# jordi-adell/mcarray

Hardware: AMD Instinct MI355X
Metric: STFT frames/sec, 8-mic GCC-PHAT + SRP-PHAT(361) + delay-and-sum beamform @48kHz/1024-pt (higher is better)
Workload: dtype f32 (SRP operands adaptive); 1 GPU; BASELINE configs[2] geometry (8-mic ULA 0.04 m, 48 kHz, N=1024, hop 512, 361 angles, 1 source, no power floor), 8 arrays x 4096 frames per GPU per step; channel rows padded by 64 floats; arrays_per_gpu=8, frames_per_array=4096, srp_precision=adaptive, parallelism=arrays sharded over 1 GPU(s), all_gather of DOA bins+prob

## Files before the change

__graft_entry__.py:

```python
import os
import subprocess
import sys

ROOT = os.path.dirname(os.path.abspath(__file__))
if ROOT not in sys.path:
    sys.path.insert(0, ROOT)


def build():
    env = dict(os.environ)
    subprocess.check_call(["make", "-C", os.path.join(ROOT, "mcarray_amd", "csrc"), "-j4", "-s"], env=env)
    subprocess.check_call(["make", "-C", os.path.join(ROOT, "oracle"), "-s"], env=env)
    cxx = os.path.join(ROOT, "tests", "cxx", "Makefile")
    if os.path.exists(cxx):
        subprocess.check_call(["make", "-C", os.path.dirname(cxx), "-s"], env=env)
    import mcarray_amd
    from mcarray_amd import _lib
    _lib.load()


def smoke():
    import numpy as np
    from mcarray_amd import api, synth
    from oracle import pyoracle as po
    fs, N, F = 48000, 1024, 12
    xs = synth.ULA8
    pcm = synth.noise_source_stream(xs, np.deg2rad(23.0), fs, (F + 1) * N // 2, 42)
    ctx = api.Context(fs, xs, N, 0.5, 1, srp_precision=api.SRP_FP32, device=0)
    r = ctx.process_frames_host(pcm[None], want_energy=True)
    o = po.ssl_stream(fs, N, xs, pcm.astype(np.float64), 1, 0.5, want_map=True)
    assert np.array_equal(r["bin"][0], o["bin"]), (r["bin"][0].T, o["bin"].T)
    assert np.abs(r["energy"][0] - o["energy"]).max() <= 2e-5 * np.abs(o["energy"]).max()
    assert np.abs(r["out"][0] - o["out"]).max() <= 2e-5 * np.abs(o["out"]).max() + 1e-7
    print("smoke ok: DOA bins", r["bin"][0, :, 0].tolist(), "->", float(np.rad2deg(r["doa"][0, -1, 0])), "deg")


if __name__ == "__main__":
    build()
    if len(sys.argv) > 1 and sys.argv[1] == "smoke":
        smoke()
```

mcarray_amd/csrc/api.hip:

```cpp
#include "../../include/mcarray_hip.h"
#include "fft1024c.h"
#include "kernels.h"
#include "knobs.h"
#include "stage.h"

#include <chrono>
#include <cmath>
#include <cstdio>
#include <cstdlib>
#include <cstring>
#include <string>
#include <thread>
#include <vector>

using namespace mca;

namespace {

std::string g_create_error;

struct TimedEvent { int id; hipEvent_t a, b; };

}

struct mca_hip_graph;

#define MCA_MAX_LANES 1

constexpr int FB_LAG = 2, FB_RING = 64, FB_WAIT_MS = 4000;
struct Knobs {
    bool fb_enabled = true;
    long long adapt_min_rows = 4096;
    int adapt_max_sources = 1;
    double tau_scale = 1.0;
// ... 28 lines not shown
    {
        auto F = [](void *q) { if (q) (void)hipFree(q); };
        F(d_A); F(d_Ax); F(d_C); F(d_Cx); F(d_part); F(d_estart); F(d_nv); F(d_power); F(d_voiced); F(d_power_out);
        F(d_flags); F(d_chunk_from); F(d_list); F(d_need); F(d_umask); F(d_nlist); F(d_last_vchunk); F(d_unsure);
        *this = Workspace();
    }
};

struct G2FrameState {
    double power_floor = 0, samples = 0, noise_estimated = 0;
    double silence = 0;
    double corr_mem = 0, doa_mem = 0;
    double doa = 0, prob = -1;
};

struct mca_hip_ctx {
    mca_hip_config cfg{};
    std::vector<double> xyz;
    int M = 0, P = 0, G = 0, D = 0, Dp = 0, K = 0, N = 0, H = 0, logH = 0, Kp = 0, S = 1, prec = 0;
    bool ula = false, stream_ok = false, generic = false;
    bool n512 = false;
    bool n2048 = false;
    std::string stream_why;
    float step = 0.f;
    std::vector<float> delays, grid;
    std::vector<int2> pairs;
    float *d_window = nullptr, *d_grid = nullptr, *d_delays = nullptr;
    float2 *d_tw = nullptr;
    double *d_micx = nullptr;
    int2 *d_pairs = nullptr;
    void *d_B = nullptr, *d_Bt = nullptr;
    bool merged = false; int n_merged = 0, Kp_m = 0;
    void *d_Bm = nullptr, *d_Btm = nullptr; unsigned short *d_mrank = nullptr;
    float2 *d_bftab = nullptr; int bf_pairs = 0;
    float4 *d_steer_rows = nullptr; float2 *d_steer_q = nullptr; float *d_steer_nyq = nullptr; int *d_steer_pred = nullptr; unsigned long long *d_steer_miss = nullptr;
    float2 *d_steer_Y = nullptr; size_t steer_Y_rows = 0; float *d_steer_tail = nullptr;
    int *d_steer_mlist = nullptr;
    bool steer_now = false, steer_fused_now = false;
    bool steer_mlist_dirty = false;
    bool steer_patched_now = false;
    unsigned long long steer_frames_total = 0, steer_fused_calls = 0;
    unsigned long long *h_steer = nullptr;
    unsigned long long steer_seq = 0, steer_seq_seen = 0, steer_call_frames[FB_RING] = {};
    bool steer_spec = true, steer_lost = false;
    float *d_E[2] = {nullptr, nullptr};
    float *d_tail[2] = {nullptr, nullptr};
    int e_cur = 0, tail_cur = 0;
    Workspace lanes[MCA_MAX_LANES];
    int cur_lane = 0, a0 = 0;
    long long plan_rows = 0;
    int plan_arrays = 0;
    int n_lanes_last = 1;
    hipStream_t io_stream[3] = {}; hipEvent_t io_ev[8] = {};
    Workspace &ws() { return lanes[cur_lane]; }
    double *d_gate_state = nullptr;
    int *d_last_bin = nullptr; float *d_last_rad = nullptr, *d_last_prob = nullptr;
    int last_arrays = 0, last_frames = 0;
    float *d_doa[2] = {nullptr, nullptr};
    int doa_cur = 0;
    long long gcc2_frames_done = 0;
    long long *d_vdone[2] = {nullptr, nullptr};
    int *d_g2_vidx = nullptr, *d_g2_nv = nullptr; float *d_g2_rad = nullptr, *d_g2_prob = nullptr; size_t g2_rows = 0;
    unsigned char *d_g2_reset = nullptr;
    int *d_g2_post0 = nullptr;
    int *d_silence = nullptr;
    bool tracked = false;
// ... 51 lines not shown
namespace {

int fail(mca_hip_ctx *c, int code, const std::string &msg)
{
    if (c) c->err = msg; else g_create_error = msg;
    return code;
}

#define HIP_TRY(ctx, expr)                                                                              \
    do {                                                                                                \
        hipError_t _e = (expr);                                                                         \
        if (_e != hipSuccess)                                                                           \
            return fail(ctx, _e == hipErrorOutOfMemory ? MCA_HIP_ERR_OUT_OF_MEMORY : MCA_HIP_ERR_HIP,   \
                        std::string(#expr) + ": " + hipGetErrorString(_e));                            \
    } while (0)

double speed_of_sound() { return 346.1; }
float doa_idx2angle(int idx, float step) { float pr = (float)idx * step; return (float)((double)pr - M_PI_2); }
float doa_to_delay_far_field(float doa, float microDist)
{
    return (float)(((double)microDist * std::sin((double)doa)) / speed_of_sound());
}
float doa_to_delay_samples(float doa, float microDist, int fs) { return doa_to_delay_far_field(doa, microDist) * (float)fs; }
double distance(const std::vector<double> &xyz, int i, int j)
{
    return std::sqrt(std::pow(xyz[3 * j] - xyz[3 * i], 2) + std::pow(xyz[3 * j + 1] - xyz[3 * i + 1], 2) +
                     std::pow(xyz[3 * j + 2] - xyz[3 * i + 2], 2));
}

void free_ctx(mca_hip_ctx *c)
{
    if (!c) return;
    auto F = [](void *p) { if (p) (void)hipFree(p); };
    F(c->d_window); F(c->d_tw); F(c->d_grid); F(c->d_delays); F(c->d_micx); F(c->d_pairs); F(c->d_B); F(c->d_Bt); F(c->d_bftab); F(c->d_steer_rows); F(c->d_steer_q); F(c->d_steer_nyq); F(c->d_steer_pred); F(c->d_steer_miss); F(c->d_steer_Y); F(c->d_steer_mlist); F(c->d_steer_tail); F(c->d_Bm); F(c->d_Btm); F(c->d_mrank);
    F(c->d_E[0]); F(c->d_E[1]); F(c->d_tail[0]); F(c->d_tail[1]); F(c->d_doa[0]); F(c->d_doa[1]); F(c->d_vdone[0]); F(c->d_vdone[1]); F(c->d_g2_vidx); F(c->d_g2_nv); F(c->d_g2_rad); F(c->d_g2_prob);
    F(c->d_g2_reset); F(c->d_g2_post0); F(c->d_silence);
    F(c->d_trk_x); F(c->d_trk_sd); F(c->d_trk_si); F(c->d_trk_sil); F(c->d_trk_corr); F(c->d_trk_idx); F(c->d_trk_res);
    F(c->d_rstats); F(c->d_gate_state);
    for (int i = 0; i < 2; ++i) { F(c->d_hist_pcm[i]); F(c->d_hist_C[i]); F(c->d_ehist[i]); }
    if (c->h_probe) (void)hipHostFree(c->h_probe);
    if (c->h_steer) (void)hipHostFree(c->h_steer);
    for (Workspace &w : c->lanes) w.release();
    for (auto &e : c->io_ev) if (e) (void)hipEventDestroy(e);
    for (auto &q : c->io_stream) if (q) (void)hipStreamDestroy(q);
    F(c->d_last_bin); F(c->d_last_rad); F(c->d_last_prob);
    F(c->d_fr); F(c->d_E64[0]); F(c->d_E64[1]); F(c->d_res); F(c->d_bins); F(c->d_out64);
    F(c->d_g2f_corr[0]); F(c->d_g2f_corr[1]); F(c->d_g2f_res);
    c->stage.release();
    for (auto &e : c->events) { (void)hipEventDestroy(e.a); (void)hipEventDestroy(e.b); }
    for (auto &e : c->pool) (void)hipEventDestroy(e);
    delete c;
}

int round_up(int v, int m) { return (v + m - 1) / m * m; }

Knobs read_knobs(const mca_hip_config &cfg)
{
    Knobs k;
    auto geti = [](const char *v, long long dflt) { return v ? std::atoll(v) : dflt; };
    k.fb_enabled = cfg.adaptive_fallback != MCA_HIP_ADAPT_FALLBACK_OFF;
    if (const char *v = env_str("MCA_HIP_ADAPT_FALLBACK")) k.fb_enabled = std::atoi(v) != 0;
    k.adapt_min_rows = geti(env_str("MCA_HIP_ADAPT_MIN_ROWS"), cfg.adaptive_min_rows > 0 ? cfg.adaptive_min_rows : 4096);
    k.adapt_max_sources = (int)geti(env_str("MCA_HIP_ADAPT_MAX_SOURCES"), cfg.adaptive_max_sources > 0 ? cfg.adaptive_max_sources : 1);
    if (const char *v = env_str("MCA_HIP_ADAPT_TAU_SCALE")) k.tau_scale = std::atof(v);
    if (const char *v = env_str("MCA_HIP_WS_MAX_MB")) k.ws_max_bytes = (long long)std::atoll(v) << 20;
    k.force_generic = env_str("MCA_HIP_FORCE_GENERIC") != nullptr;
    k.scan_carry = cfg.scan_carry != 0 || env_str("MCA_HIP_SCAN_CARRY") != nullptr;
// ... 47 lines not shown
                        _Float16 hi = (_Float16)v[q];
                        B[(size_t)d * Kp + kk] = hi;
                        if (planes == 2) B[((size_t)Dp + d) * Kp + kk] = (_Float16)(v[q] - (float)hi);
                    }
                }
        HIP_TRY(c, hipMalloc(&c->d_B, B.size() * sizeof(_Float16)));
        HIP_TRY(c, hipMemcpy(c->d_B, B.data(), B.size() * sizeof(_Float16), hipMemcpyHostToDevice));
        if (Dp == 384) {
            const int ns32 = Kp / 32;
            std::vector<_Float16> Bt(B.size());
            for (int pl = 0; pl < planes; ++pl)
                for (int sl = 0; sl < ns32; ++sl)
                    for (int d = 0; d < Dp; ++d)
                        std::memcpy(&Bt[(((size_t)pl * ns32 + sl) * Dp + d) * 32], &B[((size_t)pl * Dp + d) * Kp + (size_t)sl * 32], 32 * sizeof(_Float16));
            HIP_TRY(c, hipMalloc(&c->d_Bt, Bt.size() * sizeof(_Float16)));
            HIP_TRY(c, hipMemcpy(c->d_Bt, Bt.data(), Bt.size() * sizeof(_Float16), hipMemcpyHostToDevice));
        }
    }
    return MCA_HIP_OK;
}

int cur_kp(const mca_hip_ctx *c) { return (c->merged && c->a_planes == 1) ? c->Kp_m : c->Kp; }

int build_merged_tables(mca_hip_ctx *c)
{
    c->merged = false;
    if (!c->ula || (c->generic && !c->n2048) || c->n512 || (c->M != 4 && c->M != 8) || c->Dp % 64 != 0) return MCA_HIP_OK;
    if (c->prec != MCA_HIP_SRP_ADAPTIVE && c->prec != MCA_HIP_SRP_FP16) return MCA_HIP_OK;
    const int K = c->K, D = c->D, Dp = c->Dp, G = c->G;
    const double N = 2.0 * (K - 1);
    for (int g = 1; g < G; ++g)
        for (int d = 0; d < D; ++d)
            if (std::fabs((double)c->delays[(size_t)g * D + d] - (g + 1) * (double)c->delays[d]) > 1e-4) return MCA_HIP_OK;
    std::vector<unsigned short> rank((size_t)G * (K - 1) + 1, 0xffff);
    std::vector<int> ms;
    for (int g = 1; g <= G; ++g)
        for (int k = 0; k < K; ++k) rank[(size_t)k * g] = 0;
    for (size_t m = 0; m < rank.size(); ++m)
        if (rank[m] == 0) { rank[m] = (unsigned short)ms.size(); ms.push_back((int)m); }
    c->n_merged = (int)ms.size();
    c->Kp_m = round_up(2 * ((c->n_merged + 63) & ~63), 32);
    const int Kp = c->Kp_m;
    std::vector<_Float16> B((size_t)Dp * Kp, (_Float16)0.f);
    for (int d = 0; d < D; ++d)
        for (int r = 0; r < c->n_merged; ++r) {
            const double ph = 2.0 * M_PI * (double)ms[(size_t)r] * (double)c->delays[d] / N;
            B[(size_t)d * Kp + 2 * r] = (_Float16)(float)std::cos(ph);
            B[(size_t)d * Kp + 2 * r + 1] = (_Float16)(float)(-std::sin(ph));
        }
    HIP_TRY(c, hipMalloc(&c->d_Bm, B.size() * sizeof(_Float16)));
    HIP_TRY(c, hipMemcpy(c->d_Bm, B.data(), B.size() * sizeof(_Float16), hipMemcpyHostToDevice));
    if (Dp == 384) {
        const int ns32 = Kp / 32;
        std::vector<_Float16> Bt(B.size());
        for (int sl = 0; sl < ns32; ++sl)
            for (int d = 0; d < Dp; ++d)
                std::memcpy(&Bt[((size_t)sl * Dp + d) * 32], &B[(size_t)d * Kp + (size_t)sl * 32], 32 * sizeof(_Float16));
        HIP_TRY(c, hipMalloc(&c->d_Btm, Bt.size() * sizeof(_Float16)));
        HIP_TRY(c, hipMemcpy(c->d_Btm, Bt.data(), Bt.size() * sizeof(_Float16), hipMemcpyHostToDevice));
    }
    rank.resize((rank.size() + 3) / 4 * 4, 0xffff);
    HIP_TRY(c, hipMalloc((void **)&c->d_mrank, rank.size() * sizeof(unsigned short)));
    HIP_TRY(c, hipMemcpy(c->d_mrank, rank.data(), rank.size() * sizeof(unsigned short), hipMemcpyHostToDevice));
    c->merged = true;
    c->a_row_elems = cur_kp(c) * c->a_planes;
    return MCA_HIP_OK;
}

void time_begin(mca_hip_ctx *c, int id, hipStream_t st)
{
    c->timing_open = (c->timing >> id) & 1u;
    if (!c->timing_open) return;
    TimedEvent ev; ev.id = id;
    auto get = [&]() { hipEvent_t e; if (!c->pool.empty()) { e = c->pool.back(); c->pool.pop_back(); } else (void)hipEventCreate(&e); return e; };
    ev.a = get(); ev.b = get();
    (void)hipEventRecord(ev.a, st);
    c->events.push_back(ev);
}
void time_end(mca_hip_ctx *c, hipStream_t st)
{
    if (!c->timing_open) return;
    c->timing_open = false;
    (void)hipEventRecord(c->events.back().b, st);
}

int gen_threads(const mca_hip_ctx *c, bool synthesis)
{
    if (c->N >= 4096) return 1024;
    if (c->N >= 2048) return synthesis ? 512 : 1024;
    return 256;
}

struct GemmPlan { bool v2; int ksplit; };
GemmPlan plan_gemm(const mca_hip_ctx *c, long long rows)
{
    GemmPlan g;
    if (c->plan_rows > 0) rows = c->plan_rows;
    const long long deep = cur_kp(c) >= 12288 ? 2 : 1;
    g.v2 = c->prec != MCA_HIP_SRP_FP32 && c->Dp == 384 && rows * (c->a_planes == 2 ? deep : 1) >= 16384LL * (c->a_planes == 2 ? 2 : 1);
    if (g.v2) {
        g.ksplit = rows >= 65536 ? 1 : (rows >= 32768 || cur_kp(c) < 6144 ? 2 : 4);
    } else {
        const long long wgs = (rows + 127) / 128 * (c->Dp == 64 ? 1 : c->Dp / 192);
        const int nk = cur_kp(c) / (c->prec == MCA_HIP_SRP_FP32 ? 16 : 32);
        long long ks = 512 / (wgs > 0 ? wgs : 1);
        if (ks > nk / 8) ks = nk / 8;
        if (ks > 16) ks = 16;
        if (ks < 1) ks = 1;
        g.ksplit = (int)ks;
    }
    return g;
}

void *&a_buf(mca_hip_ctx *c) { return (c->prec == MCA_HIP_SRP_ADAPTIVE && c->a_planes == 2) ? c->ws().d_Ax : c->ws().d_A; }
size_t &a_buf_bytes(mca_hip_ctx *c) { return (c->prec == MCA_HIP_SRP_ADAPTIVE && c->a_planes == 2) ? c->ws().ax_bytes : c->ws().a_bytes; }

int ensure_a(mca_hip_ctx *c, long long rows)
{
    size_t need_a = (size_t)((rows + 255) / 256 * 256) * c->a_row_elems * c->a_elem;
    void *&buf = a_buf(c); size_t &bytes = a_buf_bytes(c);
    if (need_a > bytes) {
        if (buf) (void)hipFree(buf);
        buf = nullptr; bytes = 0;
        HIP_TRY(c, hipMalloc(&buf, need_a));
        HIP_TRY(c, hipMemset(buf, 0, need_a));
        HIP_TRY(c, hipDeviceSynchronize());
        bytes = need_a; ++c->ws_gen;
    }
    return MCA_HIP_OK;
}

int ensure_workspace(mca_hip_ctx *c, long long rows_chunk, long long rows_total)
{
    int rc_a = ensure_a(c, rows_chunk);
    if (rc_a) return rc_a;
    const int planes = std::max(2, plan_gemm(c, rows_chunk).ksplit);
    size_t need_c = (size_t)rows_total * c->Dp * sizeof(float) * planes;
    if (need_c > c->ws().c_bytes) {
        if (c->ws().d_C) (void)hipFree(c->ws().d_C);
        c->ws().d_C = nullptr; c->ws().c_bytes = 0;
        HIP_TRY(c, hipMalloc((void **)&c->ws().d_C, need_c));
        c->ws().c_bytes = need_c; ++c->ws_gen;
    }
// ... 795 lines not shown
    c->cur_lane = 0;
    return reserve_lane(c, n_arrays, n_frames);
}

int mca_hip_reserve(mca_hip_ctx *c, int n_arrays, int n_frames)
{
    if (!c || n_arrays < 1 || n_frames < 1) return MCA_HIP_ERR_INVALID_ARGUMENT;
    const int rc = reserve_impl(c, n_arrays, n_frames);
    return rc ? rc : steer_reserve(c, n_arrays, n_frames);
}

static int run_correlation_map(mca_hip_ctx *c, const float *pcm, long long array_stride, long long mic_stride,
                               int n_arrays, int n_frames, hipStream_t st)
{
    int rc;
    const long long fc = chunk_frames_for(c, n_arrays, n_frames);
    if ((rc = ensure_workspace(c, (long long)n_arrays * fc, (long long)n_arrays * n_frames))) return rc;
    if ((rc = ensure_scan_workspace(c, n_arrays, n_frames, (n_frames + SCAN_CHUNK - 1) / SCAN_CHUNK))) return rc;
    bool fused_partial = SCAN_CHUNK == 32 && c->a_planes == 1 && !c->cfg.use_power_floor && n_frames % SCAN_CHUNK == 0 && fc % SCAN_CHUNK == 0 &&
                         plan_gemm(c, (long long)n_arrays * fc).ksplit <= 2;
    for (int f0 = 0; fused_partial && f0 < n_frames; f0 += (int)fc)
        fused_partial = plan_gemm(c, (long long)n_arrays * std::min<long long>(fc, n_frames - f0)).v2;
    c->ws().partial_done = fused_partial;
    c->ws().part_planes = fused_partial ? plan_gemm(c, (long long)n_arrays * fc).ksplit : 1;
    for (int f0 = 0; f0 < n_frames; f0 += (int)fc) {
        const int nf = (int)std::min<long long>(fc, n_frames - f0);
        StftPhatArgs sa{};
        sa.pcm = pcm; sa.array_stride = array_stride; sa.mic_stride = mic_stride;
        sa.M = c->M; sa.n_frames = nf; sa.frame0 = f0;
        sa.fpb = 16;
        while (sa.fpb > 1 && (long long)n_arrays * ((nf + sa.fpb - 1) / sa.fpb) < 256) sa.fpb >>= 1;
        sa.power = c->cfg.use_power_floor ? c->ws().d_power : nullptr; sa.total_frames = n_frames;
        sa.window = c->d_window; sa.A = a_buf(c); sa.Kp = c->Kp; sa.a_row_elems = c->a_row_elems; sa.a_planes = c->a_planes;
        if (c->merged && c->a_planes == 1) { sa.mrank = c->d_mrank; sa.n_merged = c->n_merged; }
        sa.N = c->N; sa.logH = c->logH; sa.kg = c->K; sa.ula = c->ula ? 1 : 0; sa.tw = c->d_tw;
        sa.no_phat = c->cfg.gcc_weighting == MCA_HIP_GCC_NONE ? 1 : 0;
        if (c->prec == MCA_HIP_SRP_ADAPTIVE && c->a_planes == 1 && wave16_applies(c)) sa.unsure = c->ws().d_unsure;
        if (c->lazy_now && cand_call(c, true)) sa.dead = c->ws().d_unsure;
        if (c->lazy_now) sa.hist_out = c->d_hist_pcm[c->hist_cur ^ 1];
        if (c->steer_now && sa.mrank && !sa.power) {
            sa.bf.rows = c->d_steer_rows; sa.bf.q = c->d_steer_q; sa.bf.nyq = c->d_steer_nyq; sa.bf.pred = c->d_steer_pred + c->a0; sa.bf.Y = c->d_steer_Y;
        }
        time_begin(c, MCA_HIP_K_STFT_PHAT, st);
        if (c->n512) {
            rc = c->prec == MCA_HIP_SRP_FP32 ? launch_stft_512<float>(c, sa, dim3(0, n_arrays), st) : launch_stft_512<_Float16>(c, sa, dim3(0, n_arrays), st);
        } else if ((c->N == 4096 || c->N == 2048) && c->M == 2 && c->stream_ok) {
            sa.fpb = 8;
            while (sa.fpb > 2 && (long long)n_arrays * ((nf + sa.fpb - 1) / sa.fpb) < 512) sa.fpb >>= 1;
            const size_t smem4 = ((size_t)16 * 258 + 8 * FFT_SCRATCH + TW_WIN) * sizeof(float2) + 4 * 8 * sizeof(float);
            dim3 g4((nf + sa.fpb - 1) / sa.fpb, n_arrays);
#define LSUB(RR, T)                                                                                                       \
            do {                                                                                                          \
                HIP_TRY(c, hipFuncSetAttribute(reinterpret_cast<const void *>(&k_stft_phat_sub2<RR, T>), hipFuncAttributeMaxDynamicSharedMemorySize, (int)smem4)); \
                hipLaunchKernelGGL((k_stft_phat_sub2<RR, T>), g4, dim3(512), smem4, st, sa);                              \
            } while (0)
            if (c->N == 4096) { if (c->prec == MCA_HIP_SRP_FP32) LSUB(8, float); else LSUB(8, _Float16); }
            else { if (c->prec == MCA_HIP_SRP_FP32) LSUB(4, float); else LSUB(4, _Float16); }
#undef LSUB
            rc = MCA_HIP_OK;
        } else if (n2048_analysis(c)) {
            rc = c->prec == MCA_HIP_SRP_FP32 ? launch_stft_2048<float>(c, sa, dim3(0, n_arrays), st) : launch_stft_2048<_Float16>(c, sa, dim3(0, n_arrays), st);
        } else if (c->generic) {
            const size_t smem1 = (size_t)c->M * (c->H + 1) * sizeof(float2) + 16;
#define GEN_LAUNCH(K)                                                                                                     \
            do {                                                                                                          \
                if (smem1 > 64 * 1024)                                                                                    \
                    HIP_TRY(c, hipFuncSetAttribute(reinterpret_cast<const void *>(&K), hipFuncAttributeMaxDynamicSharedMemorySize, (int)smem1)); \
                hipLaunchKernelGGL(K, dim3(nf, n_arrays), dim3(gen_threads(c, false)), smem1, st, sa);                                      \
            } while (0)
            if (c->prec == MCA_HIP_SRP_FP32) GEN_LAUNCH(k_stft_phat_gen<float>);
            else GEN_LAUNCH(k_stft_phat_gen<_Float16>);
#undef GEN_LAUNCH
            rc = MCA_HIP_OK;
        } else {
            dim3 g1((nf + sa.fpb - 1) / sa.fpb, n_arrays);
            const size_t smem1 = ((size_t)c->M * FFT_SCRATCH + TW_WORDS + (size_t)sa.fpb * c->M) * sizeof(float2) + (size_t)sa.fpb * 8 * sizeof(float);
            rc = c->prec == MCA_HIP_SRP_FP32 ? launch_stft<float>(c, sa, g1, smem1, st) : launch_stft<_Float16>(c, sa, g1, smem1, st);
        }
        time_end(c, st);
        if (rc) return rc;

        GemmArgs ga{};
        const bool mg = c->merged && c->a_planes == 1;
        ga.A = a_buf(c); ga.B = mg ? c->d_Bm : c->d_B; ga.C = c->ws().d_C; ga.Bt = mg ? c->d_Btm : c->d_Bt;
        ga.rows = n_arrays * nf; ga.chunk_frames = nf; ga.total_frames = n_frames; ga.frame0 = f0;
        ga.Kp = cur_kp(c); ga.Dp = c->Dp; ga.a_row_elems = c->a_row_elems;
        ga.c_plane_elems = (long long)n_arrays * n_frames * c->Dp;
        if (fused_partial) {
            ga.part = c->ws().d_part; ga.nvoiced = c->ws().d_nv; ga.D = c->D; ga.n_chunks = n_frames / SCAN_CHUNK;
            ga.part_plane_stride = (long long)n_arrays * ga.n_chunks * c->D;
            ga.scan_w[31] = 1 - 0.8f;
            for (int t = 30; t >= 0; --t) ga.scan_w[t] = ga.scan_w[t + 1] * 0.8f;
        }
        const bool v2 = plan_gemm(c, ga.rows).v2;
        const int ksplit = plan_gemm(c, (long long)n_arrays * fc).ksplit;
        c->ws().c_planes = ksplit; c->ws().c_plane = ga.c_plane_elems;
        time_begin(c, MCA_HIP_K_SRP_GEMM, st);
        if (v2) {
            const int np = c->a_planes;
            const size_t smem = (size_t)(np == 2 ? 2 : 4) * np * (256 + 384) * 64;
            dim3 gv((ga.rows + 255) / 256, ksplit);
#define V2_LAUNCH(K)                                                                                                      \
            do {                                                                                                          \
                HIP_TRY(c, hipFuncSetAttribute(reinterpret_cast<const void *>(&K), hipFuncAttributeMaxDynamicSharedMemorySize, (int)smem)); \
                hipLaunchKernelGGL(K, gv, dim3(512), smem, st, ga);                                                       \
            } while (0)
            if (c->a_planes == 2) V2_LAUNCH(k_srp_gemm_f16_v2);
            else V2_LAUNCH(k_srp_gemm_f16_v3);
#undef V2_LAUNCH
        } else {
            dim3 g2((ga.rows + 127) / 128, c->Dp == 64 ? 1 : c->Dp / 192, ksplit);
            if (c->prec == MCA_HIP_SRP_FP32) hipLaunchKernelGGL(k_srp_gemm_f32, g2, dim3(256), 0, st, ga);
            else if (c->Dp == 64 && c->a_planes == 2) hipLaunchKernelGGL((k_srp_gemm_f16<true, 64>), g2, dim3(256), 0, st, ga);
            else if (c->Dp == 64) hipLaunchKernelGGL((k_srp_gemm_f16<false, 64>), g2, dim3(256), 0, st, ga);
            else if (c->a_planes == 2) hipLaunchKernelGGL((k_srp_gemm_f16<true, 192>), g2, dim3(256), 0, st, ga);
            else hipLaunchKernelGGL((k_srp_gemm_f16<false, 192>), g2, dim3(256), 0, st, ga);
        }
        time_end(c, st);
        HIP_TRY(c, hipGetLastError());
    }
    if (c->ws().c_planes > 2) {
        const long long n4 = c->ws().c_plane / 4;
        time_begin(c, MCA_HIP_K_FOLD, st);
        hipLaunchKernelGGL(k_sum_planes, dim3((unsigned)((n4 + 255) / 256)), dim3(256), 0, st, c->ws().d_C, n4, c->ws().c_planes, c->ws().c_plane);
        time_end(c, st);
        HIP_TRY(c, hipGetLastError());
        c->ws().c_planes = 1;
    }

    return MCA_HIP_OK;
}

constexpr float ENERGY_MU = 0.8f, ENERGY_ONE_MINUS_MU = 1 - 0.8f;

static void launch_repair_contraction(mca_hip_ctx *c, Workspace &w, long long list0, long long pass_rows, int ksplit_arrays, RepairPatchArgs pp, hipStream_t st)
{
    GemmArgs ga{};
    ga.A = w.d_Ax; ga.B = c->d_B; ga.C = w.d_Cx; ga.Bt = c->d_Bt;
    ga.rows = (int)pass_rows; ga.chunk_frames = (int)pass_rows; ga.total_frames = (int)pass_rows; ga.frame0 = 0;
    ga.Kp = c->Kp; ga.Dp = c->Dp; ga.a_row_elems = c->a_row_elems; ga.c_plane_elems = pass_rows * c->Dp;
// ... 1399 lines not shown
```

mcarray_amd/csrc/kernels.h:

```cpp
#pragma once
#include "mca_internal.h"

namespace mca {

template <int MT, bool ULA, typename OutT> __global__ void k_stft_phat(StftPhatArgs p);
template <int MT, bool ULA, typename OutT> __global__ void k_stft_phat_few(StftPhatArgs p);
__global__ void k_sum_planes(float *C, long long n4, int planes, long long stride);
__global__ void k_scan_partial(ScanPickArgs p);
__global__ void k_scan_carry(ScanPickArgs p);
template <int PL, int MODE> __global__ void k_scan_pick(ScanPickArgs p);
template <int PL, bool PATCH> __global__ void k_scan_repick(ScanPickArgs p);
__global__ void k_repair_patch(RepairPatchArgs p);
__global__ void k_hist_list(int *list, int *n_list, int *need, int n_units);
__global__ void k_hist_settle(const float *e_hist, const float *hist_C, float *state, int *n_list, int D, int Dp, float mu, float omu);
__global__ void k_gate(GateArgs p);
__global__ void k_doa_fill(DoaFillArgs p);
template <int CPW, int OCC> __global__ void k_beamform_ola(BeamformArgs p);
template <typename OutT> __global__ void k_stft_phat_gen(StftPhatArgs p);
template <int MT, bool ULA, typename OutT> __global__ void k_stft_phat_512(StftPhatArgs p);
__global__ void k_beamform_512(BeamformArgs p);
template <int R, typename OutT> __global__ void k_stft_phat_sub2(StftPhatArgs p);
__global__ void k_beamform_gen(BeamformArgs p);
__global__ void k_bf_table(float2 *tab, const float *grid, const double *mic_x, int M, int n_pairs, double unit);
template <bool ODD> __global__ void k_beamform_wave(BeamformWaveArgs p);
template <bool POWER> __global__ void k_stft_phat_wave16(StftPhatArgs p);
template <int MT, bool ULA, typename OutT, bool MERGE = false> __global__ void k_stft_phat_2048(StftPhatArgs p);
__global__ void k_bf_table_2048(float2 *tab, const float *grid, const double *mic_x, int M, double unit);
__global__ void k_beamform_wave_2048(BeamformWaveArgs p);
template <int NPT, bool ODD> __global__ void k_beamform_wave_ms(BeamformWaveArgs p);
template <int MT, bool ULA, typename OutT, bool PL2, bool POWER, bool NOPHAT, bool MERGE, bool CAND = false, bool FUSE = false> __global__ void k_stft_phat_wave(StftPhatArgs p);
__global__ void k_steer_table(float4 *rows, float2 *q, float *nyq, const float *grid, const double *mic_x, int M, double unit);
__global__ void k_steer_patch(SteerPatchArgs p);
__global__ void k_steer_synth(SteerSynthArgs p);

__global__ void k_srp_gemm_f32(GemmArgs p);
template <bool SPLIT, int BN> __global__ void k_srp_gemm_f16(GemmArgs p);
__global__ void k_srp_gemm_f16_v2(GemmArgs p);
__global__ void k_srp_gemm_f16_v3(GemmArgs p);
template <int BN> __global__ void k_srp_gemm_repair(GemmArgs p);

template <typename T> struct C2;
template <typename T>
__global__ void k_frame_srp(const C2<T> *X, int K, int D, int P, const int2 *pairs, const float *delays,
                            const T *E_in, T *E_out, T mu, T omu, int no_phat);
template <typename T>
__global__ void k_frame_pick(const T *E, int D, int P, int S, const float *grid, T *doa, T *prob, int *bins);
template <typename T>
__global__ void k_frame_beamform(const C2<T> *X, int M, int K, int fs, const double *mic_x, double doa, C2<T> *Y);
template <typename T> __global__ void k_frame_power(const C2<T> *X, int M, int K, T *out);

__global__ void k_gcc2_scan(Gcc2ScanArgs p);
__global__ void k_gcc2_compact(const unsigned char *voiced, int n_frames, int *vidx, int *nv, const int *post0, int *silence,
                               int windows_to_decay, unsigned char *vreset);
__global__ void k_gcc2_fill(Gcc2FillArgs p);
template <typename TC, typename TA>
__global__ void k_gcc2_prob(const TC *corr, long long corr_stride, int D, float step, const float *grid, const TA *doas, TA *probs, int n);
template <typename T>
__global__ void k_frame_gcc2(const T *corr, int D, float step, const float *grid, double doa_prev, double doa_mem, double one_minus_doa_mem,
                             double *res);
template <typename TC, int SLOTS>
__global__ void k_gcc2_track(Gcc2TrackArgs p);
__global__ void k_mask_stream(MaskArgs p);
__global__ void k_mask_stream_gen(MaskGenArgs p);
__global__ void k_mask_stream_2048(MaskGenArgs p);
__global__ void k_mask_frame(MaskFrameArgs p);
__global__ void k_mb_analyse(MbAnalyseArgs p);
__global__ void k_mb_analyse_1024(MbAnalyseArgs p, int fpb);
__global__ void k_mb_analyse_512(MbAnalyseArgs p, int fpb);
__global__ void k_mb_scan(MbScanArgs p);
__global__ void k_mb_summary(MbSummaryArgs p);
__global__ void k_mvdr_analyse(MvdrAnalyseArgs p);
// ... 31 lines not shown
```

mcarray_amd/csrc/kernels_gemm.hip:

```cpp
#include "mca_internal.h"

namespace mca {

typedef float f32x16 __attribute__((ext_vector_type(16)));
typedef _Float16 f16x8 __attribute__((ext_vector_type(8)));

constexpr int G32_BM = 128, G32_BN = 192, G32_BK = 16;

__global__ __launch_bounds__(256) void k_srp_gemm_f32(GemmArgs p)
{
    __shared__ float As[G32_BK][G32_BM + 4];
    __shared__ float Bs[G32_BK][G32_BN + 4];
    const int tid = threadIdx.x, lane = tid & 63, wave = tid >> 6;
    const int wm = wave >> 1, wn = wave & 1;
    const int row0 = blockIdx.x * G32_BM, col0 = blockIdx.y * G32_BN;
    const float *A = reinterpret_cast<const float *>(p.A);
    const float *B = reinterpret_cast<const float *>(p.B);

    f32x16 acc[2][3];
#pragma unroll
    for (int i = 0; i < 2; ++i)
#pragma unroll
        for (int j = 0; j < 3; ++j)
#pragma unroll
// ... 410 lines not shown
        float wt[2][4];
#pragma unroll
        for (int b2 = 0; b2 < 2; ++b2)
#pragma unroll
            for (int r = 0; r < 4; ++r) {
                const int g4 = lane >> 4;
                const float w01 = g4 == 0 ? p.scan_w[b2 * 16 + r] : p.scan_w[b2 * 16 + 4 + r];
                const float w23 = g4 == 2 ? p.scan_w[b2 * 16 + 8 + r] : p.scan_w[b2 * 16 + 12 + r];
                wt[b2][r] = g4 < 2 ? w01 : w23;
            }
#pragma unroll
        for (int ch = 0; ch < 2; ++ch) {
            const int frow0 = row0 + wm * 64 + ch * 32;
            if (frow0 < p.rows) {
                const int arr = frow0 / p.chunk_frames, chunk = (p.frame0 + frow0 - arr * p.chunk_frames) >> 5;
                float *out = p.part + blockIdx.y * p.part_plane_stride + ((long long)arr * p.n_chunks + chunk) * p.D + wn * 192 + (lane & 15);
#pragma unroll
                for (int j = 0; j < 12; ++j) {
                    float sacc = 0.f;
#pragma unroll
                    for (int b2 = 0; b2 < 2; ++b2)
#pragma unroll
                        for (int r = 0; r < 4; ++r) sacc = fmaf(wt[b2][r], acc[2 * ch + b2][j][r], sacc);
                    sacc += __shfl_xor(sacc, 16);
                    sacc += __shfl_xor(sacc, 32);
                    if (lane < 16 && wn * 192 + j * 16 + lane < p.D) out[j * 16] = sacc;
                }
                if (wn == 0 && lane == 0 && blockIdx.y == 0) p.nvoiced[(long long)arr * p.n_chunks + chunk] = 32;
            }
        }
    }
}

}
```

mcarray_amd/csrc/kernels_wave.hip:

```cpp
#include <type_traits>

#include "fft1024c.h"
#include "mca_internal.h"
#include "cand_unit.h"
#include "phat_pairs.h"
#include "pair_balance.h"
#include "steer.h"

namespace mca {

__global__ __launch_bounds__(256) void k_bf_table(float2 *tab, const float *grid, const double *mic_x, int M, int n_pairs, double unit)
{
    const int d = blockIdx.x, pr = blockIdx.y;
    const double doa = d == 0 ? 0.0 : (double)grid[d - 1];
    const double cd = cos(doa + 1.57079632679489661923);
    const double sc = 1.0 / ((double)M * 1024.0);
    float2 *row = tab + ((long long)d * n_pairs + pr) * 1024;
    for (int k = threadIdx.x; k < 1024; k += 256) {
        const int kap = k <= 512 ? k : k - 1024;
        double pa[2] = {0.0, 0.0}, pb[2] = {0.0, 0.0};
        for (int e = 0; e < 2; ++e) {
            const int c = 2 * pr + e;
            if (c >= M) continue;
            double turns = (double)kap * (unit * mic_x[c] * cd);
// ... 485 lines not shown
                        const uint2 o4 = offt[(2 * (g - 1) + h) * 64];
                        const unsigned off[4] = {o4.x & 0xffffu, o4.x >> 16, o4.y & 0xffffu, o4.y >> 16};
                        float2 acc[4], cur[4];
#pragma unroll
                        for (int s2 = 0; s2 < 4; ++s2) {
                            acc[s2] = make_float2(0.f, 0.f);
#pragma unroll
                            for (int i = 0; i + g < MT; ++i) acc[s2] = cmacc(acc[s2], Xh[i][4 * h + s2], Xh[i + g][4 * h + s2]);
                        }
#pragma unroll
                        for (int s2 = 0; s2 < 4; ++s2) cur[s2] = S[off[s2]];
#pragma unroll
                        for (int s2 = 0; s2 < 4; ++s2) S[off[s2]] = cadd(cur[s2], acc[s2]);
                    }
                }
                if (lane == 0) {
                    float an[MT - 1], cn[MT - 1];
                    unsigned on[MT - 1];
#pragma unroll
                    for (int g = 1; g < MT; ++g) {
                        an[g - 1] = 0.f;
#pragma unroll
                        for (int i = 0; i + g < MT; ++i) an[g - 1] = fmaf(xn[i], xn[i + g], an[g - 1]);
                        on[g - 1] = rankl[2 * (MT - 1) * 64 * 4 + g - 1];
                    }
#pragma unroll
                    for (int g = 0; g < MT - 1; ++g) cn[g] = S[on[g]].x;
#pragma unroll
                    for (int g = 0; g < MT - 1; ++g) S[on[g]].x = cn[g] + an[g];
                }
                wave_lds_fence();
                typedef _Float16 half4_t __attribute__((ext_vector_type(4)));
                typedef float float4_t __attribute__((ext_vector_type(4)));
                for (int j = lane; j < nmp / 2; j += 64) {
                    const float4 v = reinterpret_cast<const float4 *>(S)[j];
                    const float4_t vv = {v.x, v.y, v.z, v.w};
                    reinterpret_cast<half4_t *>(arow)[j] = __builtin_convertvector(vv, half4_t);
                }
                wave_lds_fence();
            } else {
#pragma unroll
                for (int s = 0; s < 8; ++s) {
                    if constexpr (ULA) {
                        float2 r[MT], out[NOUT];
#pragma unroll
                        for (int m = 0; m < MT; ++m) r[m] = Xh[m][s];
                        pair_products<MT, ULA>(r, out);
#pragma unroll
                        for (int g = 0; g < NOUT; ++g) store_a_wave<PL2>(arow, voff, g * KG + 64 * s, out[g], p.Kp);
                    } else {
                        int pi = 0;
#pragma unroll
                        for (int i = 0; i < MT; ++i)
#pragma unroll
                            for (int j = i + 1; j < MT; ++j) { store_a_wave<PL2>(arow, voff, pi * KG + 64 * s, cmulc(Xh[i][s], Xh[j][s]), p.Kp); ++pi; }
                    }
                }
            }
            if (POWER) {
                const float pacc = wave_sum64(ptime.x + ptime.y);
                if (lane == 0) p.power[(long long)a * p.total_frames + p.frame0 + f] = pacc / (float)FFT_N / (float)MT;
            }
        }
        wave_lds_fence();
        if (!MERGE && lane < f_end - f_begin) {
            float2 xn[MT], out[NOUT];
// ... 350 lines not shown
```

mcarray_amd/csrc/mca_internal.h:

```cpp
#pragma once
#include <hip/hip_runtime.h>

#define MCA_MAX_SOURCES 4
#define MCA_MAX_MICS 16

namespace mca {

constexpr int MK_NB = 4;
constexpr int MK_WARM = 8;
constexpr int BF_NB = 4;
constexpr int GCC2_DOAWARM = 64;
constexpr int SCAN_WARM = 96;
constexpr int KG = 513;
#ifndef MCA_SCAN_CHUNK
#define MCA_SCAN_CHUNK 32
#endif
#ifndef MCA_SCAN_SUB
#define MCA_SCAN_SUB 32
#endif
constexpr int SCAN_CHUNK = MCA_SCAN_CHUNK;
constexpr int SCAN_SUB = MCA_SCAN_SUB;
#ifndef MCA_SCAN_LD
#define MCA_SCAN_LD 8
#endif
// ... 39 lines not shown
    int f0, f1;
    const float *window;
    const int *doa_bin;
    SteerArgs bf;
    int y_f0, y_frames;
    int all;
    unsigned long long *miss;
};
struct SteerSynthArgs {
    const float2 *Y; int n_frames, f0, f1, ft, y_f0, y_frames;
    float *out;
    const float *tail_in; float *tail_out;
    const int *doa_bin; int *pred_out;
    unsigned long long *report; unsigned long long seq; unsigned long long *miss_total;
    int *n_miss;
};

struct StftPhatArgs {
    const float *pcm;
    long long array_stride, mic_stride;
    int M, n_frames, frame0, fpb;
    const float *window;
    void *A;
    int Kp;
    int a_row_elems;
    int a_planes;
    float *power;
    int total_frames;
    int N, logH, kg, ula;
    const float2 *tw;
    const int *list; const int *n_list; int list0, list_cap, groups_per_array;
    float *hist_out; const float *hist_in; int hist_base;
    const unsigned short *mrank; int n_merged;
    int no_phat;
    int skew;
    unsigned char *dead;
    unsigned char *unsure;
    int cand_on; CandArgs cand;
    SteerArgs bf;
};

__device__ __forceinline__ void store_a(float *row, const StftPhatArgs &, int cidx, float2 v)
{
    reinterpret_cast<float2 *>(row)[cidx] = v;
}

typedef _Float16 half2_t __attribute__((ext_vector_type(2)));

typedef float float2_t __attribute__((ext_vector_type(2)));

__device__ __forceinline__ void store_a(_Float16 *row, const StftPhatArgs &p, int cidx, float2 v)
{
    const float2_t vv = {v.x, v.y};
    const half2_t hi = __builtin_convertvector(vv, half2_t);
    reinterpret_cast<half2_t *>(row)[cidx] = hi;
    if (p.a_planes == 2) {
        const float2_t back = __builtin_convertvector(hi, float2_t);
        const half2_t lo = __builtin_convertvector(vv - back, half2_t);
        reinterpret_cast<half2_t *>(row + p.Kp)[cidx] = lo;
    }
}

struct GemmArgs {
    const void *A;
    const void *B;
    float *C;
    int rows;
    int chunk_frames, total_frames, frame0;
    int Kp, Dp, a_row_elems;
    long long c_plane_elems;
    const void *Bt;
    const int *n_list; int list0;
    int repair_ksplit;
    int repair_items;
    float *part; int *nvoiced; int D, n_chunks;
    long long part_plane_stride;
    float scan_w[32];
};

struct ScanPickArgs {
    const float *C;
    int c_planes; long long c_plane_stride;
    int n_frames, Dp, D, P, S, chunk, n_chunks;
    float mu, one_minus_mu;
    float inv_norm;
    const float *state_in;
    float *state_out;
    float *part;
    int part_planes; long long part_plane_stride;
    int *nvoiced;
    float *e_start;
    const unsigned char *voiced;
    const float *grid;
    int *doa_bin; float *doa_rad; float *prob; float *energy;
    int mode;
    float tau;
    unsigned char *flags;
    int groups_per_array;
    int *need;
    int *list;
    int *n_list;
    int *chunk_from;
    int *clist; int *n_clist;
    int lookback;
    unsigned long long *probe;
    unsigned long long probe_seq;
    int *last_vchunk;
// ... 454 lines not shown
```

Baseline: 57.90 million frames/s.

## Fold symmetric SRP steering columns into half-width fp16 GEMM

Adds a folded SRP GEMM path for ULA geometries whose steering delays are antisymmetric about the center angle. The merged spectral products are stored planar (real then imaginary halves), so the real plane times cosine gives the even part and the imaginary plane times sine gives the odd part. Each is computed on a separate y-plane over only (D+1)/2 columns, and the epilogue mirrors results to both angles with a sign flip. This roughly halves the B-matrix columns and MFMA work, at the cost of a new kernel, new host tables, a changed A layout in the STFT kernel, and dependence on the exact plan conditions (ksplit==2, Dp==384).

```diff
diff --git a/__graft_entry__.py b/__graft_entry__.py
--- a/__graft_entry__.py
+++ b/__graft_entry__.py
@@ -14,6 +14,9 @@
     cxx = os.path.join(ROOT, "tests", "cxx", "Makefile")
     if os.path.exists(cxx):
         subprocess.check_call(["make", "-C", os.path.dirname(cxx), "-s"], env=env)
+    harness = os.path.join(ROOT, "tests", "cxx", "gemm_harness.mk")
+    if os.path.exists(harness):
+        subprocess.check_call(["make", "-C", os.path.dirname(harness), "-f", "gemm_harness.mk", "-s"], env=env)
     import mcarray_amd
     from mcarray_amd import _lib
     _lib.load()
diff --git a/mcarray_amd/csrc/api.hip b/mcarray_amd/csrc/api.hip
--- a/mcarray_amd/csrc/api.hip
+++ b/mcarray_amd/csrc/api.hip
@@ -1,5 +1,6 @@
 #include "../../include/mcarray_hip.h"
 #include "fft1024c.h"
+#include "fold_table.h"
 #include "kernels.h"
 #include "knobs.h"
 #include "stage.h"
@@ -94,6 +95,7 @@
     void *d_B = nullptr, *d_Bt = nullptr;
     bool merged = false; int n_merged = 0, Kp_m = 0;
     void *d_Bm = nullptr, *d_Btm = nullptr; unsigned short *d_mrank = nullptr;
+    bool fold = false; void *d_Bfold = nullptr;
     float2 *d_bftab = nullptr; int bf_pairs = 0;
     float4 *d_steer_rows = nullptr; float2 *d_steer_q = nullptr; float *d_steer_nyq = nullptr; int *d_steer_pred = nullptr; unsigned long long *d_steer_miss = nullptr;
     float2 *d_steer_Y = nullptr; size_t steer_Y_rows = 0; float *d_steer_tail = nullptr;
@@ -211,7 +213,7 @@
 {
     if (!c) return;
     auto F = [](void *p) { if (p) (void)hipFree(p); };
-    F(c->d_window); F(c->d_tw); F(c->d_grid); F(c->d_delays); F(c->d_micx); F(c->d_pairs); F(c->d_B); F(c->d_Bt); F(c->d_bftab); F(c->d_steer_rows); F(c->d_steer_q); F(c->d_steer_nyq); F(c->d_steer_pred); F(c->d_steer_miss); F(c->d_steer_Y); F(c->d_steer_mlist); F(c->d_steer_tail); F(c->d_Bm); F(c->d_Btm); F(c->d_mrank);
+    F(c->d_window); F(c->d_tw); F(c->d_grid); F(c->d_delays); F(c->d_micx); F(c->d_pairs); F(c->d_B); F(c->d_Bt); F(c->d_bftab); F(c->d_steer_rows); F(c->d_steer_q); F(c->d_steer_nyq); F(c->d_steer_pred); F(c->d_steer_miss); F(c->d_steer_Y); F(c->d_steer_mlist); F(c->d_steer_tail); F(c->d_Bm); F(c->d_Btm); F(c->d_Bfold); F(c->d_mrank);
     F(c->d_E[0]); F(c->d_E[1]); F(c->d_tail[0]); F(c->d_tail[1]); F(c->d_doa[0]); F(c->d_doa[1]); F(c->d_vdone[0]); F(c->d_vdone[1]); F(c->d_g2_vidx); F(c->d_g2_nv); F(c->d_g2_rad); F(c->d_g2_prob);
     F(c->d_g2_reset); F(c->d_g2_post0); F(c->d_silence);
     F(c->d_trk_x); F(c->d_trk_sd); F(c->d_trk_si); F(c->d_trk_sil); F(c->d_trk_corr); F(c->d_trk_idx); F(c->d_trk_res);
@@ -325,15 +327,25 @@
     for (int g = 1; g < G; ++g)
         for (int d = 0; d < D; ++d)
             if (std::fabs((double)c->delays[(size_t)g * D + d] - (g + 1) * (double)c->delays[d]) > 1e-4) return MCA_HIP_OK;
-    std::vector<unsigned short> rank((size_t)G * (K - 1) + 1, 0xffff);
+    std::vector<unsigned short> rank;
     std::vector<int> ms;
-    for (int g = 1; g <= G; ++g)
-        for (int k = 0; k < K; ++k) rank[(size_t)k * g] = 0;
-    for (size_t m = 0; m < rank.size(); ++m)
-        if (rank[m] == 0) { rank[m] = (unsigned short)ms.size(); ms.push_back((int)m); }
+    merged_products(G, K, rank, ms);
     c->n_merged = (int)ms.size();
     c->Kp_m = round_up(2 * ((c->n_merged + 63) & ~63), 32);
     const int Kp = c->Kp_m;
+    c->fold = fold_applies(true, c->N, FFT_N, D, Dp, c->delays.data());
+    if (c->fold) {
+        FoldTables ft;
+        build_fold_tables(c->delays.data(), D, Dp, ms.data(), c->n_merged, Kp, c->N, ft);
+        auto up16 = [&](void **dst, const std::vector<uint16_t> &v, size_t at, size_t total) {
+            if (!*dst) HIP_TRY(c, hipMalloc(dst, total * 2));
+            HIP_TRY(c, hipMemcpy((char *)*dst + at * 2, v.data(), v.size() * 2, hipMemcpyHostToDevice));
+            return (int)MCA_HIP_OK;
+        };
+        int rc;
+        if ((rc = up16(&c->d_Bm, ft.full, 0, ft.full.size())) || (rc = up16(&c->d_Btm, ft.full_tiled, 0, ft.full_tiled.size())) ||
+            (rc = up16(&c->d_Bfold, ft.even, 0, 2 * ft.even.size())) || (rc = up16(&c->d_Bfold, ft.odd, ft.even.size(), 2 * ft.even.size()))) return rc;
+    } else {
     std::vector<_Float16> B((size_t)Dp * Kp, (_Float16)0.f);
     for (int d = 0; d < D; ++d)
         for (int r = 0; r < c->n_merged; ++r) {
@@ -352,6 +364,7 @@
         HIP_TRY(c, hipMalloc(&c->d_Btm, Bt.size() * sizeof(_Float16)));
         HIP_TRY(c, hipMemcpy(c->d_Btm, Bt.data(), Bt.size() * sizeof(_Float16), hipMemcpyHostToDevice));
     }
+    }
     rank.resize((rank.size() + 3) / 4 * 4, 0xffff);
     HIP_TRY(c, hipMalloc((void **)&c->d_mrank, rank.size() * sizeof(unsigned short)));
     HIP_TRY(c, hipMemcpy(c->d_mrank, rank.data(), rank.size() * sizeof(unsigned short), hipMemcpyHostToDevice));
@@ -384,7 +397,7 @@
     return 256;
 }
 
-struct GemmPlan { bool v2; int ksplit; };
+struct GemmPlan { bool v2; int ksplit; bool fold; };
 GemmPlan plan_gemm(const mca_hip_ctx *c, long long rows)
 {
     GemmPlan g;
@@ -402,6 +415,7 @@
         if (ks < 1) ks = 1;
         g.ksplit = (int)ks;
     }
+    g.fold = g.v2 && g.ksplit == 2 && c->a_planes == 1 && c->merged && c->fold;
     return g;
 }
 
@@ -1263,7 +1277,7 @@
         while (sa.fpb > 1 && (long long)n_arrays * ((nf + sa.fpb - 1) / sa.fpb) < 256) sa.fpb >>= 1;
         sa.power = c->cfg.use_power_floor ? c->ws().d_power : nullptr; sa.total_frames = n_frames;
         sa.window = c->d_window; sa.A = a_buf(c); sa.Kp = c->Kp; sa.a_row_elems = c->a_row_elems; sa.a_planes = c->a_planes;
-        if (c->merged && c->a_planes == 1) { sa.mrank = c->d_mrank; sa.n_merged = c->n_merged; }
+        if (c->merged && c->a_planes == 1) { sa.mrank = c->d_mrank; sa.n_merged = c->n_merged; sa.planar = c->fold ? 1 : 0; }
         sa.N = c->N; sa.logH = c->logH; sa.kg = c->K; sa.ula = c->ula ? 1 : 0; sa.tw = c->d_tw;
         sa.no_phat = c->cfg.gcc_weighting == MCA_HIP_GCC_NONE ? 1 : 0;
         if (c->prec == MCA_HIP_SRP_ADAPTIVE && c->a_planes == 1 && wave16_applies(c)) sa.unsure = c->ws().d_unsure;
@@ -1317,6 +1331,7 @@
         ga.rows = n_arrays * nf; ga.chunk_frames = nf; ga.total_frames = n_frames; ga.frame0 = f0;
         ga.Kp = cur_kp(c); ga.Dp = c->Dp; ga.a_row_elems = c->a_row_elems;
         ga.c_plane_elems = (long long)n_arrays * n_frames * c->Dp;
+        ga.Bf = mg ? c->d_Bfold : nullptr; ga.D = c->D;
         if (fused_partial) {
             ga.part = c->ws().d_part; ga.nvoiced = c->ws().d_nv; ga.D = c->D; ga.n_chunks = n_frames / SCAN_CHUNK;
             ga.part_plane_stride = (long long)n_arrays * ga.n_chunks * c->D;
@@ -1337,6 +1352,11 @@
                 hipLaunchKernelGGL(K, gv, dim3(512), smem, st, ga);                                                       \
             } while (0)
             if (c->a_planes == 2) V2_LAUNCH(k_srp_gemm_f16_v2);
+            else if (ksplit == 2 && mg && c->fold) {
+                const size_t smem_f = (size_t)FOLD_NS * (256 + 192) * 64;
+                HIP_TRY(c, hipFuncSetAttribute(reinterpret_cast<const void *>(&k_srp_gemm_f16_fold), hipFuncAttributeMaxDynamicSharedMemorySize, (int)smem_f));
+                hipLaunchKernelGGL(k_srp_gemm_f16_fold, gv, dim3(512), smem_f, st, ga);
+            }
             else V2_LAUNCH(k_srp_gemm_f16_v3);
 #undef V2_LAUNCH
         } else {
diff --git a/mcarray_amd/csrc/fold_table.h b/mcarray_amd/csrc/fold_table.h
--- /dev/null
+++ b/mcarray_amd/csrc/fold_table.h
@@ -0,0 +1,83 @@
+#pragma once
+#include <cmath>
+#include <cstdint>
+#include <cstring>
+#include <vector>
+
+namespace mca {
+
+constexpr int FOLD_DP = 384, FOLD_COLS = 192;
+constexpr double FOLD_MAX_ASYM = 4e-6;
+
+inline uint16_t f16_bits(float f)
+{
+    uint32_t x;
+    std::memcpy(&x, &f, 4);
+    const uint16_t sign = (uint16_t)((x >> 16) & 0x8000u);
+    x &= 0x7fffffffu;
+    if (x > 0x7f800000u) return sign | 0x7e00u;
+    if (x >= 0x477ff000u) return sign | 0x7c00u;
+    if (x < 0x38800000u) {
+        float a;
+        std::memcpy(&a, &x, 4);
+        a += 0.5f;
+        std::memcpy(&x, &a, 4);
+        return sign | (uint16_t)(x - 0x3f000000u);
+    }
+    const uint32_t odd = (x >> 13) & 1u;
+    x += ((uint32_t)(15 - 127) << 23) + 0xfffu + odd;
+    return sign | (uint16_t)(x >> 13);
+}
+
+inline void merged_products(int G, int K, std::vector<unsigned short> &rank, std::vector<int> &ms)
+{
+    rank.assign((size_t)G * (K - 1) + 1, 0xffff);
+    ms.clear();
+    for (int g = 1; g <= G; ++g)
+        for (int k = 0; k < K; ++k) rank[(size_t)k * g] = 0;
+    for (size_t m = 0; m < rank.size(); ++m)
+        if (rank[m] == 0) { rank[m] = (unsigned short)ms.size(); ms.push_back((int)m); }
+}
+
+inline bool fold_applies(bool merged, int n_frame, int fft_n, int D, int Dp, const float *delay)
+{
+    if (!merged || n_frame != fft_n || Dp != FOLD_DP || D < 3 || (D & 1) == 0) return false;
+    const int c = (D - 1) / 2;
+    if (c >= FOLD_COLS) return false;
+    for (int j = 0; j <= c; ++j)
+        if (!(std::fabs((double)delay[c + j] + (double)delay[c - j]) <= FOLD_MAX_ASYM)) return false;
+    return true;
+}
+
+inline double fold_delay(const float *delay, int c, int j) { return j == 0 ? (double)delay[c] : 0.5 * ((double)delay[c + j] - (double)delay[c - j]); }
+
+struct FoldTables {
+    int c = 0, half = 0;
+    std::vector<uint16_t> even, odd;
+    std::vector<uint16_t> full;
+    std::vector<uint16_t> full_tiled;
+};
+
+inline void build_fold_tables(const float *delay, int D, int Dp, const int *ms, int n_merged, int Kp, int n_frame, FoldTables &t)
+{
+    const int c = (D - 1) / 2, half = Kp / 2, ns = half / 32;
+    t.c = c; t.half = half;
+    t.even.assign((size_t)ns * FOLD_COLS * 32, 0); t.odd.assign((size_t)ns * FOLD_COLS * 32, 0);
+    t.full.assign((size_t)Dp * Kp, 0); t.full_tiled.assign((size_t)Dp * Kp, 0);
+    for (int j = 0; j <= c; ++j) {
+        const double tj = fold_delay(delay, c, j);
+        for (int r = 0; r < n_merged; ++r) {
+            const double ph = 2.0 * M_PI * (double)ms[r] * tj / (double)n_frame;
+            const uint16_t cs = f16_bits((float)std::cos(ph)), sn = f16_bits((float)(-std::sin(ph)));
+            const size_t e = ((size_t)(r >> 5) * FOLD_COLS + j) * 32 + (r & 31);
+            t.even[e] = cs; t.odd[e] = sn;
+            t.full[(size_t)(c + j) * Kp + r] = cs; t.full[(size_t)(c + j) * Kp + half + r] = sn;
+            if (j > 0) { t.full[(size_t)(c - j) * Kp + r] = cs; t.full[(size_t)(c - j) * Kp + half + r] = (sn & 0x7fffu) ? (uint16_t)(sn ^ 0x8000u) : sn; }
+        }
+    }
+    for (int sl = 0; sl < Kp / 32; ++sl)
+        for (int d = 0; d < Dp; ++d)
+            std::memcpy(&t.full_tiled[((size_t)sl * Dp + d) * 32], &t.full[(size_t)d * Kp + (size_t)sl * 32], 32 * sizeof(uint16_t));
+}
+
+}
diff --git a/mcarray_amd/csrc/kernels.h b/mcarray_amd/csrc/kernels.h
--- a/mcarray_amd/csrc/kernels.h
+++ b/mcarray_amd/csrc/kernels.h
@@ -37,6 +37,7 @@
 template <bool SPLIT, int BN> __global__ void k_srp_gemm_f16(GemmArgs p);
 __global__ void k_srp_gemm_f16_v2(GemmArgs p);
 __global__ void k_srp_gemm_f16_v3(GemmArgs p);
+__global__ void k_srp_gemm_f16_fold(GemmArgs p);
 template <int BN> __global__ void k_srp_gemm_repair(GemmArgs p);
 
 template <typename T> struct C2;
diff --git a/mcarray_amd/csrc/kernels_gemm.hip b/mcarray_amd/csrc/kernels_gemm.hip
--- a/mcarray_amd/csrc/kernels_gemm.hip
+++ b/mcarray_amd/csrc/kernels_gemm.hip
@@ -466,4 +466,151 @@
     }
 }
 
-}
+__global__ __launch_bounds__(512) void k_srp_gemm_f16_fold(GemmArgs p)
+{
+    constexpr int BN = 192;
+    constexpr int A_BYTES = V2_BM * V3_ROWB, B_BYTES = BN * V3_ROWB;
+    constexpr int STAGE = A_BYTES + B_BYTES;
+    constexpr int NS = FOLD_NS;
+    extern __shared__ __attribute__((aligned(1024))) unsigned char smem_g[];
+    const int tid = threadIdx.x, lane = tid & 63, wave = __builtin_amdgcn_readfirstlane(tid >> 6);
+    const int wm = wave >> 1, wn = wave & 1;
+    const int row0 = blockIdx.x * V2_BM, y = blockIdx.y;
+    const int half = p.Kp / 2, ns = half / V3_BK;
+    const unsigned char *A = reinterpret_cast<const unsigned char *>(p.A);
+    const unsigned char *B = reinterpret_cast<const unsigned char *>(p.Bf) + (long long)y * ns * B_BYTES;
+    const bool b2 = wave < 4;
+
+    const int lrow = lane >> 2, pch = lane & 3;
+    const int r0 = wave * 16 + lrow;
+    const int lch = pch ^ v3_swz(r0);
+    const unsigned char *a_lane = A + ((long long)(row0 + r0) * p.a_row_elems + (long long)y * half + lch * 8) * 2;
+    const unsigned char *b_lane = B + r0 * V3_ROWB + lch * 16;
+    const long long a_blk = (long long)128 * p.a_row_elems * 2;
+    const int dst0 = wave * 1024;
+
+    f32x4 acc[4][6];
+#pragma unroll
+    for (int i = 0; i < 4; ++i)
+#pragma unroll
+        for (int j = 0; j < 6; ++j)
+#pragma unroll
+            for (int r = 0; r < 4; ++r) acc[i][j][r] = 0.f;
+
+    auto issue_a = [&](int s, int buf) {
+        const long long koff_a = (long long)s * V3_BK * 2;
+        unsigned char *sb = smem_g + buf * STAGE;
+#pragma unroll
+        for (int i = 0; i < 2; ++i)
+            __builtin_amdgcn_global_load_lds(reinterpret_cast<const void *>(a_lane + i * a_blk + koff_a), (lds_void_t *)(sb + dst0 + i * 8192), 16, 0, 0);
+    };
+    auto issue_b = [&](int s, int buf) {
+        const long long koff_b = (long long)s * B_BYTES;
+        unsigned char *sb = smem_g + buf * STAGE;
+        __builtin_amdgcn_global_load_lds(reinterpret_cast<const void *>(b_lane + koff_b), (lds_void_t *)(sb + A_BYTES + dst0), 16, 0, 0);
+        if (b2) __builtin_amdgcn_global_load_lds(reinterpret_cast<const void *>(b_lane + 128 * V3_ROWB + koff_b), (lds_void_t *)(sb + A_BYTES + dst0 + 8192), 16, 0, 0);
+    };
+
+    const int ra = wm * 64 + (lane & 15), rb = wn * 96 + (lane & 15);
+    const int a_off0 = ra * V3_ROWB + (((lane >> 4) ^ v3_swz(ra)) << 4);
+    const int b_off0 = rb * V3_ROWB + (((lane >> 4) ^ v3_swz(rb)) << 4);
+    const unsigned lds0 = (unsigned)(uintptr_t)((lds_void_t *)smem_g);
+
+#pragma unroll
+    for (int q = 0; q < NS - 1; ++q)
+        if (q < ns) { issue_a(q, q); issue_b(q, q); }
+    for (int s = 0; s < ns; ++s) {
+        const int later = min(NS - 2, ns - 1 - s);
+        if (b2) {
+            if (later >= 2) asm volatile("s_waitcnt vmcnt(8)" ::: "memory");
+            else if (later == 1) asm volatile("s_waitcnt vmcnt(4)" ::: "memory");
+            else asm volatile("s_waitcnt vmcnt(0)" ::: "memory");
+        } else {
+            if (later >= 2) asm volatile("s_waitcnt vmcnt(6)" ::: "memory");
+            else if (later == 1) asm volatile("s_waitcnt vmcnt(3)" ::: "memory");
+            else asm volatile("s_waitcnt vmcnt(0)" ::: "memory");
+        }
+        __builtin_amdgcn_s_barrier();
+        const bool more = s + NS - 1 < ns;
+        if (more) issue_a(s + NS - 1, (s + NS - 1) % NS);
+#define LDS_RD(dst, addr, off) asm volatile("ds_read_b128 %0, %1 offset:%2" : "=v"(dst) : "v"(addr), "n"(off))
+        f16x8 af[4], bs[2];
+        const unsigned a_addr = lds0 + (s % NS) * STAGE + a_off0;
+        const unsigned b_addr = lds0 + (s % NS) * STAGE + A_BYTES + b_off0;
+        LDS_RD(af[0], a_addr, 0); LDS_RD(af[1], a_addr, 1024); LDS_RD(af[2], a_addr, 2048); LDS_RD(af[3], a_addr, 3072);
+        LDS_RD(bs[0], b_addr, 0); LDS_RD(bs[1], b_addr, 1024);
+#pragma unroll
+        for (int j = 0; j < 6; ++j) {
+            if (j == 5 && more) issue_b(s + NS - 1, (s + NS - 1) % NS);
+            if (j == 0) asm volatile("s_waitcnt lgkmcnt(1)" : "+v"(af[0]), "+v"(af[1]), "+v"(af[2]), "+v"(af[3]), "+v"(bs[0]));
+            else if (j < 5) asm volatile("s_waitcnt lgkmcnt(1)" : "+v"(bs[j % 2]));
+            else asm volatile("s_waitcnt lgkmcnt(0)" : "+v"(bs[j % 2]));
+#pragma unroll
+            for (int i = 0; i < 4; ++i) acc[i][j] = __builtin_amdgcn_mfma_f32_16x16x32_f16(af[i], bs[j % 2], acc[i][j], 0, 0, 0);
+            __builtin_amdgcn_sched_barrier(0);
+            if (j + 2 < 6) LDS_RD(bs[j % 2], b_addr, (j + 2) * 1024);
+            __builtin_amdgcn_sched_barrier(0);
+        }
+#undef LDS_RD
+    }
+    const int cc = (p.D - 1) / 2, npad = p.Dp - p.D, jj0 = wn * 96 + (lane & 15);
+    float *Cp = p.C + (long long)y * p.c_plane_elems;
+#pragma unroll
+    for (int i = 0; i < 4; ++i)
+#pragma unroll
+        for (int r = 0; r < 4; ++r) {
+            const int frow = row0 + wm * 64 + i * 16 + 4 * (lane >> 4) + r;
+            if (frow < p.rows) {
+                const int arr = frow / p.chunk_frames, fl = frow - arr * p.chunk_frames;
+                float *crow = Cp + ((long long)arr * p.total_frames + p.frame0 + fl) * p.Dp;
+#pragma unroll
+                for (int j = 0; j < 6; ++j) {
+                    const int jj = jj0 + j * 16;
+                    const float v = acc[i][j][r];
+                    if (jj <= cc) {
+                        crow[cc + jj] = v;
+                        if (jj > 0) crow[cc - jj] = y ? -v : v;
+                    }
+                    if (jj < npad) crow[p.D + jj] = 0.f;
+                }
+            }
+        }
+    if (p.part) {
+        float wt[2][4];
+#pragma unroll
+        for (int b = 0; b < 2; ++b)
+#pragma unroll
+            for (int r = 0; r < 4; ++r) {
+                const int g4 = lane >> 4;
+                const float w01 = g4 == 0 ? p.scan_w[b * 16 + r] : p.scan_w[b * 16 + 4 + r];
+                const float w23 = g4 == 2 ? p.scan_w[b * 16 + 8 + r] : p.scan_w[b * 16 + 12 + r];
+                wt[b][r] = g4 < 2 ? w01 : w23;
+            }
+#pragma unroll
+        for (int ch = 0; ch < 2; ++ch) {
+            const int frow0 = row0 + wm * 64 + ch * 32;
+            if (frow0 < p.rows) {
+                const int arr = frow0 / p.chunk_frames, chunk = (p.frame0 + frow0 - arr * p.chunk_frames) >> 5;
+                float *out = p.part + y * p.part_plane_stride + ((long long)arr * p.n_chunks + chunk) * p.D;
+#pragma unroll
+                for (int j = 0; j < 6; ++j) {
+                    float sacc = 0.f;
+#pragma unroll
+                    for (int b = 0; b < 2; ++b)
+#pragma unroll
+                        for (int r = 0; r < 4; ++r) sacc = fmaf(wt[b][r], acc[2 * ch + b][j][r], sacc);
+                    sacc += __shfl_xor(sacc, 16);
+                    sacc += __shfl_xor(sacc, 32);
+                    const int jj = jj0 + j * 16;
+                    if (lane < 16 && jj <= cc) {
+                        out[cc + jj] = sacc;
+                        if (jj > 0) out[cc - jj] = y ? -sacc : sacc;
+                    }
+                }
+                if (wn == 0 && lane == 0 && y == 0) p.nvoiced[(long long)arr * p.n_chunks + chunk] = 32;
+            }
+        }
+    }
+}
+
+}
diff --git a/mcarray_amd/csrc/kernels_wave.hip b/mcarray_amd/csrc/kernels_wave.hip
--- a/mcarray_amd/csrc/kernels_wave.hip
+++ b/mcarray_amd/csrc/kernels_wave.hip
@@ -541,6 +541,14 @@
                 wave_lds_fence();
                 typedef _Float16 half4_t __attribute__((ext_vector_type(4)));
                 typedef float float4_t __attribute__((ext_vector_type(4)));
+                if (p.planar) {
+                    for (int j = lane; j < nmp / 4; j += 64) {
+                        const float4 v0 = reinterpret_cast<const float4 *>(S)[2 * j], v1 = reinterpret_cast<const float4 *>(S)[2 * j + 1];
+                        const float4_t re = {v0.x, v0.z, v1.x, v1.z}, im = {v0.y, v0.w, v1.y, v1.w};
+                        reinterpret_cast<half4_t *>(arow)[j] = __builtin_convertvector(re, half4_t);
+                        reinterpret_cast<half4_t *>(arow + nmp)[j] = __builtin_convertvector(im, half4_t);
+                    }
+                } else
                 for (int j = lane; j < nmp / 2; j += 64) {
                     const float4 v = reinterpret_cast<const float4 *>(S)[j];
                     const float4_t vv = {v.x, v.y, v.z, v.w};
diff --git a/mcarray_amd/csrc/mca_internal.h b/mcarray_amd/csrc/mca_internal.h
--- a/mcarray_amd/csrc/mca_internal.h
+++ b/mcarray_amd/csrc/mca_internal.h
@@ -95,6 +95,7 @@
     const int *list; const int *n_list; int list0, list_cap, groups_per_array;
     float *hist_out; const float *hist_in; int hist_base;
     const unsigned short *mrank; int n_merged;
+    int planar;
     int no_phat;
     int skew;
     unsigned char *dead;
@@ -123,6 +124,8 @@
         reinterpret_cast<half2_t *>(row + p.Kp)[cidx] = lo;
     }
 }
+
+constexpr int FOLD_NS = 4;
 
 struct GemmArgs {
     const void *A;
@@ -136,6 +139,7 @@
     const int *n_list; int list0;
     int repair_ksplit;
     int repair_items;
+    const void *Bf;
     float *part; int *nvoiced; int D, n_chunks;
     long long part_plane_stride;
     float scan_w[32];
```

Result: faster. 59.91 million frames/s, median of 6 (+3.5%).
